# mdolab/adflow

Measured on NVIDIA H100. Metric: Mcells/s RANS-SA residual, higher is better.
Workload: dtype f64

## Files before the change

adflow_b200/csrc/adflow_b200.cu:

```cuda
#include <cuda_runtime.h>
#include <math.h>
#include <stdarg.h>
#include <stdio.h>
#include <string.h>

#include <map>
#include <string>
#include <vector>
#include <algorithm>

#include "adfb_common.cuh"
#include "state_kernels.cuh"
#include "residual_kernels.cuh"
#include "smoother_kernels.cuh"
#include "mg_kernels.cuh"
#include "ank_kernels.cuh"
#include "krylov_kernels.cuh"
#include "halo_kernels.cuh"
#include "dadi_kernels.cuh"
#include "sa_kernels.cuh"

namespace {

struct Block {
// ... 920 lines not shown
    static int mode = -1;
    if (mode < 0) { const char* e = getenv("ADFB_L2_PERSIST"); mode = e ? atoi(e) : 0; }
    static const void* current = nullptr;
    Block* only = nullptr;
    int nAlive = 0;
    for (Block& b : g.blocks) if (b.alive) { only = &b; nAlive++; }
    const void* want = (mode && nAlive == 1) ? (const void*)only->dev.w : nullptr;
    if (want == current) return;
    current = want;
    cudaStreamAttrValue av;
    memset(&av, 0, sizeof av);
    if (want) {
        int dev = 0, maxWin = 0, l2 = 0;
        cudaGetDevice(&dev);
        cudaDeviceGetAttribute(&maxWin, cudaDevAttrMaxAccessPolicyWindowSize, dev);
        cudaDeviceGetAttribute(&l2, cudaDevAttrMaxPersistingL2CacheSize, dev);
        size_t bytes = only->slabBytes;
        if ((size_t)maxWin < bytes) bytes = (size_t)maxWin;
        cudaDeviceSetLimit(cudaLimitPersistingL2CacheSize, (size_t)l2 < bytes ? (size_t)l2 : bytes);
        av.accessPolicyWindow.base_ptr = (void*)want;
        av.accessPolicyWindow.num_bytes = bytes;
        av.accessPolicyWindow.hitRatio = ((size_t)l2 >= bytes) ? 1.0f : (float)l2 / (float)bytes;
        av.accessPolicyWindow.hitProp = cudaAccessPropertyPersisting;
        av.accessPolicyWindow.missProp = cudaAccessPropertyStreaming;
    } else {
        av.accessPolicyWindow.num_bytes = 0;
    }
    cudaStreamSetAttribute(g.stream, cudaStreamAttributeAccessPolicyWindow, &av);
    cudaGetLastError();
}

static int residual_body(int level, unsigned flags) {
    static int overlapOn = -1;
    if (overlapOn < 0) { const char* e = getenv("ADFB_OVERLAP_BC"); overlapOn = e ? atoi(e) : 0; }
    static cudaStream_t s2 = nullptr;
    static cudaEvent_t eFork = nullptr, eJoin = nullptr;
    const bool preamble = !(flags & ADFB_RES_SKIP_PREAMBLE);
    const bool overlap = overlapOn && preamble && !g_kt.on && !overset_present(level);
    if (overlap && !s2) {
        CK(cudaStreamCreateWithFlags(&s2, cudaStreamNonBlocking));
        CK(cudaEventCreateWithFlags(&eFork, cudaEventDisableTiming));
        CK(cudaEventCreateWithFlags(&eJoin, cudaEventDisableTiming));
    }
    if (preamble) {
        for (Block& b : g.blocks) {
            if (!b.alive || b.level != level) continue;
            if (!g.mffdFuse && launch_state_prep(b.d, b.dev, g.prm, false, (flags & ADFB_RES_FLOW) != 0, g.stream)) return fail("state prep launch failed");
        }
        if (overlap) {
            CK(cudaEventRecord(eFork, g.stream));
            CK(cudaStreamWaitEvent(s2, eFork, 0));
            for (Block& b : g.blocks) {
                if (!b.alive || b.level != level) continue;
                if (launch_residual_core(b.d, b.dev, g.prm, flags, 1.0, 0, 1, s2, 0, RC_PREP_OWNED | RC_SA_INNER))
                    return fail("residual kernel launch failed: %s", cudaGetErrorString(cudaGetLastError()));
            }
            CK(cudaEventRecord(eJoin, s2));
        }
        const int nwLoc = g.prm.equations == ADFB_RANS ? 6 : 5;
        const bool fr = flags & ADFB_RES_FLOW, tr = (flags & ADFB_RES_TURB) && nwLoc == 6;
        const int lStart = fr ? 1 : 6, lEnd = tr ? 6 : 5;
        const bool ov = overset_present(level);
        const bool split = halo_split_ok(level);
        if (split && halo_exchange_impl(level, lStart, lEnd, 1, 1, ov, 1)) return 1;
        for (Block& b : g.blocks) {
            if (!b.alive || b.level != level) continue;
            if (launch_bc_levels(b.d, b.dev, b.subfaces, 1, g.prm.equations == ADFB_RANS && (flags & ADFB_RES_TURB), 1, g.stream))
                return fail("BC launch failed");
        }
        if (halo_exchange_impl(level, lStart, lEnd, 1, 1, ov, split ? 2 : 0)) return 1;
        if (ov) {
            for (Block& b : g.blocks) {
                if (!b.alive || b.level != level) continue;
                if (launch_bc_levels(b.d, b.dev, b.subfaces, 1, g.prm.equations == ADFB_RANS && (flags & ADFB_RES_TURB), 1, g.stream))
                    return fail("BC launch failed");
            }
        }
        if (overlap) CK(cudaStreamWaitEvent(g.stream, eJoin, 0));
    }
    const int rest = overlap ? (RC_PREP_HALO | RC_SA_SHELL | RC_FLOW) : RC_ALL;
    long long cell0 = 0;
    for (Block& b : g.blocks) {
        if (!b.alive || b.level != level) continue;
        const MffdEpi mf = {g.mffdFuse ? g.dMffd : nullptr, cell0};
        if (launch_residual_core(b.d, b.dev, g.prm, flags, 1.0, 0, 1, g.stream, 0, rest, mf))
            return fail("residual kernel launch failed: %s", cudaGetErrorString(cudaGetLastError()));
        cell0 += (long long)b.d.nx * b.d.ny * b.d.nz;
    }
    CK(cudaGetLastError());
    return 0;
}

static int nk_buffers(long long need) {
    if (g.nkN >= (size_t)need) return 0;
    for (double** p : {&g.nkA, &g.nkU, &g.nkF0, &g.nkY}) { if (*p) cudaFree(*p); *p = nullptr; }
    g.nkN = 0;
    g.nkHaveBase = false; g.ankHaveBase = false; g.ankTurbHaveBase = false;
    for (double** p : {&g.nkA, &g.nkU, &g.nkF0, &g.nkY}) CK(cudaMalloc((void**)p, need * sizeof(double)));
    if (!g.dRed) { CK(cudaMalloc((void**)&g.dRed, (2 * 1024 + 2) * sizeof(double))); g.dRedN = 2 * 1024 + 2; }
    g.nkN = need;
    return 0;
}
static int nk_vec_kernel(const double* vec, const double* base, double* out, double h, int mode) {
    long long off = 0;
    for (Block& b : g.blocks) {
        if (!b.alive || b.level != 1) continue;
        const long long n = (long long)b.d.nx * b.d.ny * b.d.nz * b.nw;
        KT_BEGIN(K_MFFD, g.stream);
        k_nkvec<<<(unsigned)((n + 255) / 256), 256, 0, g.stream>>>(b.d, b.dev, b.nw, vec ? vec + off : nullptr, base ? base + off : nullptr,
                                                                   out ? out + off : nullptr, h, mode, 0LL, LLONG_MAX);
        KT_END(K_MFFD, g.stream);
        off += n;
    }
    CK(cudaGetLastError());
    return 0;
}
static int nk_sumsq(const double* v, long long n, double* out) {
    const int nPart = 512;
    KT_BEGIN(K_MFFD, g.stream);
    k_sumsq_partial<<<nPart, 256, 0, g.stream>>>(v, n, g.dRed);
    KT_END(K_MFFD, g.stream);
    KT_BEGIN(K_MFFD, g.stream);
    k_sum_final<<<1, 256, 0, g.stream>>>(g.dRed, nPart);
    KT_END(K_MFFD, g.stream);
    if (g.nranks > 1) {
        const int rc = g.nccl.AllReduce(g.dRed + nPart, g.dRed + nPart, 1, kNcclDouble, kNcclSum, g.comm, g.stream);
        if (rc != 0) return fail("ncclAllReduce: %s", g.nccl.GetErrorString(rc));
    }
    CK(cudaMemcpyAsync(g.hRed, g.dRed + nPart, sizeof(double), cudaMemcpyDeviceToHost, g.stream));
    CK(cudaStreamSynchronize(g.stream));
    *out = g.hRed[0];
    return 0;
}
// ... 40 lines not shown
                acc += wgt[q];
                int e = (int)(acc / tot * nChunks + 0.5);
                if (e <= cb[q]) e = cb[q] + 1;
                if (e > nChunks - (S - 1 - q)) e = nChunks - (S - 1 - q);
                cb[q + 1] = e;
            }
            cb[S] = nChunks;
        }
        auto ownedEnd = [&](int chunkEnd) { return std::min(chunkEnd * kc, d.nz); };
        for (int q = 0; q < S; q++) {
            const long long q0 = (long long)ownedEnd(cb[q]) * plane, q1 = (long long)ownedEnd(cb[q + 1]) * plane;
            CK(cudaMemcpyAsync(g.nkA + off + q0, wVec + off + q0, (size_t)(q1 - q0) * sizeof(double), cudaMemcpyHostToDevice, g_ffIn));
            CK(cudaEventRecord(g_ffEv[0][q], g_ffIn));
        }
        int cNext = 0;
        for (int q = 0; q < S; q++) {
            const bool first = q == 0, last = q == S - 1;
            const int o0 = ownedEnd(cb[q]), o1 = ownedEnd(cb[q + 1]);
            CK(cudaStreamWaitEvent(sF, g_ffEv[0][q], 0));
            {
                const long long q0 = (long long)o0 * plane, q1 = (long long)o1 * plane;
                KT_BEGIN(K_MFFD, sF);
                k_nkvec<<<(unsigned)((q1 - q0 + 255) / 256), 256, 0, sF>>>(d, b.dev, b.nw, g.nkA + off, nullptr, nullptr, 0.0, 0, q0, q1);
                KT_END(K_MFFD, sF);
                dim3 tb(32, 4, 2);
                dim3 gr((d.nx + 31) / 32, (d.ny + 3) / 4, (o1 - o0 + 1) / 2);
                KT_BEGIN(K_STATE, sF);
                launch_pdl(k_state_prep, gr, tb, sF, d, b.dev, 0, rans ? 6 : 5, 1, o0, 1 + o1);
                KT_END(K_STATE, sF);
            }
            const int pLo = first ? 0 : 2 + o0, pHi = last ? d.kb : 1 + o1;
            if (launch_bc_levels(d, b.dev, b.subfaces, 1, rans ? 1 : 0, 1, sF, first ? -(1 << 30) : pLo, last ? (1 << 30) : pHi,
                                 (first ? 1 : 0) | (last ? 2 : 0)))
                return fail("BC launch failed");
            {
                dim3 tb(32, 4, 2);
                dim3 gr((d.NI + 31) / 32, (d.NJ + 3) / 4, (pHi - pLo + 2) / 2);
                KT_BEGIN(K_PREP, sF);
                launch_pdl(k_prep, gr, tb, sF, d, b.dev, 1, 1, 0, pLo, pHi);
                KT_END(K_PREP, sF);
            }
            int cEnd = cNext;
            while (cEnd < nChunks && (last || 2 + ownedEnd(cEnd + 1) - 1 + 2 <= pHi)) cEnd++;
            if (cEnd > cNext) {
                if (twoStreams) {
                    CK(cudaEventRecord(g_ffEv[2][q], sF));
                    CK(cudaStreamWaitEvent(sB, g_ffEv[2][q], 0));
                }
                const int r0 = ownedEnd(cNext), r1 = ownedEnd(cEnd);
                if (rans) {
                    dim3 tr(32, 4, 1);
                    dim3 gr((d.nx + 31) / 32, (d.ny + 3) / 4, r1 - r0);
                    KT_BEGIN(K_SA, sB);
                    k_sa<<<gr, tr, 0, sB>>>(d, b.dev, 0, MffdEpi{nullptr, 0}, r0, 1 + r1);
                    KT_END(K_SA, sB);
                }
                KT_BEGIN(K_RESID, sB);
                const int rc = launch_flowres_tile(d, b.dev, g.prm, (int)((b.dev.p - b.dev.w) / d.N), 1.0, 1, true, 0, sB, MffdEpi{nullptr, 0}, kc,
                                                   cNext, cEnd - cNext);
                KT_END(K_RESID, sB);
                if (rc) return fail("tile kernel launch failed inside the form-function pipeline");
                const long long q0 = (long long)r0 * plane, q1 = (long long)r1 * plane;
                KT_BEGIN(K_MFFD, sB);
                k_nkvec<<<(unsigned)((q1 - q0 + 255) / 256), 256, 0, sB>>>(d, b.dev, b.nw, nullptr, nullptr, g.nkY + off, 1.0, 2, q0, q1);
                KT_END(K_MFFD, sB);
                CK(cudaEventRecord(g_ffEv[1][q], sB));
                CK(cudaStreamWaitEvent(g_ffOut, g_ffEv[1][q], 0));
                CK(cudaMemcpyAsync(rVec + off + q0, g.nkY + off + q0, (size_t)(q1 - q0) * sizeof(double), cudaMemcpyDeviceToHost, g_ffOut));
                cNext = cEnd;
            }
        }
        off += (long long)d.nz * plane;
    }
    CK(cudaEventRecord(g_ffEv[3][1], g_ffIn));
    CK(cudaStreamWaitEvent(sF, g_ffEv[3][1], 0));
    CK(cudaEventRecord(g_ffEv[3][2], g_ffOut));
    CK(cudaStreamWaitEvent(sF, g_ffEv[3][2], 0));
    if (twoStreams) {
        CK(cudaEventRecord(g_ffEv[3][3], sB));
        CK(cudaStreamWaitEvent(sF, g_ffEv[3][3], 0));
    }
    CK(cudaGetLastError());
    return 0;
}
static int form_function_pipelined(const double* wVec, double* rVec, long long need) {
    (void)need;
    const int wantSlabs = form_function_pipe_slabs();
    if (wantSlabs < 2 || g.nranks > 1 || g_kt.on || g.mffdFuse) return -1;
    {
        auto busy = [](const std::map<int, Context::Pattern>& m) {
            auto it = m.find(1);
            return it != m.end() && it->second.set && (it->second.nSend || it->second.nRecv || it->second.nInt);
        };
        if (busy(g.pats) || busy(g.ovPats)) return -1;
    }
    if (!ff_pinned(wVec) || !ff_pinned(rVec)) return -1;
    for (Block& b : g.blocks) {
        if (!b.alive || b.level != 1) continue;
        if (!b.haveMetrics || b.nOrphans || !tile_kernel_applies(b.d, b.dev, g.prm) || b.d.nz < 16) return -1;
    }
    if (!g_ffIn) {
        CK(cudaStreamCreateWithFlags(&g_ffIn, cudaStreamNonBlocking));
        CK(cudaStreamCreateWithFlags(&g_ffOut, cudaStreamNonBlocking));
        CK(cudaStreamCreateWithFlags(&g_ffBack, cudaStreamNonBlocking));
        for (int a = 0; a < 4; a++) for (int q = 0; q < 34; q++) CK(cudaEventCreateWithFlags(&g_ffEv[a][q], cudaEventDisableTiming));
    }
    set_l2_window();
// ... 1101 lines not shown
```

adflow_b200/csrc/residual_kernels.cuh:

```cuda
#pragma once
#include "adfb_common.cuh"
#include <math.h>
#include <stdio.h>
#include <stdlib.h>
#include <string.h>
#include "fused_kernels.cuh"
#include "geom_cell.cuh"

#ifndef FACES_TPB
#define FACES_TPB 128
#endif
#ifndef FACES_MINB
#define FACES_MINB 4
#endif
#ifndef FACES_MINB_SPLIT
#define FACES_MINB_SPLIT 6
#endif
#ifndef SA_TPB
#define SA_TPB 128
#endif
#ifndef SA_MINB
#define SA_MINB 6
#endif
#ifndef NODAL_TPB
#define NODAL_TPB 256
#endif
#ifndef NODAL_MINB
#define NODAL_MINB 1
#endif
static inline dim3 tune_block(const char* env, dim3 dflt) {
    const char* e = getenv(env);
    if (!e) return dflt;
    int x = 0, y = 0, z = 0;
    if (sscanf(e, "%d,%d,%d", &x, &y, &z) == 3 && x > 0 && y > 0 && z > 0) return dim3(x, y, z);
    return dflt;
}

#define IRHO 0
#define IVX 1
#define IVY 2
#define IVZ 3
#define IRHOE 4
#define ITU1 5

namespace {

__global__ void __launch_bounds__(256) k_geom(Dims d, BlockDev b) {
    geom_cell(d, b, blockIdx.x * blockDim.x + threadIdx.x, blockIdx.y * blockDim.y + threadIdx.y, blockIdx.z * blockDim.z + threadIdx.z);
}

__global__ void __launch_bounds__(256) k_prep(Dims d, BlockDev b, int updateDt, int doRad, int part, int kOff, int kTop) {
    ADFB_PDL_SYNC();
    const int i = blockIdx.x * blockDim.x + threadIdx.x;
    const int j = blockIdx.y * blockDim.y + threadIdx.y;
    const int k = blockIdx.z * blockDim.z + threadIdx.z + kOff;
    if (i > d.ib || j > d.jb || k > d.kb || k > kTop) return;
    if (part) {
        const bool inner = i >= 3 && i < d.il && j >= 3 && j < d.jl && k >= 3 && k < d.kl;
        if (inner != (part == 1)) return;
    }
    const int N = (int)d.N, sJ = (int)d.sJ, sK = (int)d.sK;
    const int c = i + sJ * j + sK * k;
    const double gam = c_prm.gammaInf;
    const double rho = b.w[c], p = b.p[c];
    if (c_prm.spaceDiscr == ADFB_DISS_SCALAR) b.ss[c] = (c_prm.equations == ADFB_EULER) ? p : p * exp(-gam * log(rho));
    if (i < 1 || i > d.ie || j < 1 || j > d.je || k < 1 || k > d.ke) return;
    const bool viscous = c_prm.equations != ADFB_EULER;
    if (viscous) b.aa[c] = gam * p / rho;
    if (!doRad) return;

    const double clim2 = c_fheat[8];
    const double adis = c_prm.adis, asf = c_prm.acousticScaleFactor;
    const double ux = b.w[N + c], uy = b.w[2 * N + c], uz = b.w[3 * N + c];
    double cc2 = gam * p / rho;
    cc2 = dmax_(cc2, clim2);
    const double* ss = b.ssum;
    const double sxi = ss[c], syi = ss[N + c], szi = ss[2 * N + c];
    const double sxj = ss[3 * N + c], syj = ss[4 * N + c], szj = ss[5 * N + c];
    const double sxk = ss[6 * N + c], syk = ss[7 * N + c], szk = ss[8 * N + c];
    const double s2i = sxi * sxi + syi * syi + szi * szi;
    const double s2j = sxj * sxj + syj * syj + szj * szj;
    const double s2k = sxk * sxk + syk * syk + szk * szk;
    double ri = 0.5 * (fabs(ux * sxi + uy * syi + uz * szi) + asf * sqrt(cc2 * s2i));
    double rj = 0.5 * (fabs(ux * sxj + uy * syj + uz * szj) + asf * sqrt(cc2 * s2j));
    double rk = 0.5 * (fabs(ux * sxk + uy * syk + uz * szk) + asf * sqrt(cc2 * s2k));
    double dt = ri + rj + rk;
    if (b.coarse) {
        b.radI[c] = ri; b.radJ[c] = rj; b.radK[c] = rk;
    } else {
    ri = dmax_(ri, 1.e-25); rj = dmax_(rj, 1.e-25); rk = dmax_(rk, 1.e-25);
    const double li = log(ri), lj = log(rj), lk = log(rk);
    const double rij = exp(adis * (li - lj)), rjk = exp(adis * (lj - lk)), rik = rij * rjk;
    b.radI[c] = ri * (1.0 + 1.0 / rij + 1.0 / rik);
    b.radJ[c] = rj * (1.0 + 1.0 / rjk + rij);
    b.radK[c] = rk * (1.0 + rik + rjk);
    }

    if (!updateDt) return;
    if (i < 2 || i > d.il || j < 2 || j > d.jl || k < 2 || k > d.kl) return;
    if (viscous) {
        double rmu = b.rlv[c];
        rmu = rmu + b.rev[c];
        rmu = 0.5 * rmu / (rho * b.vol[c]);
        dt = dt + rmu * s2i;
        dt = dt + rmu * s2j;
        dt = dt + rmu * s2k;
    }
    const double plim = 0.001 * c_prm.pInfCorr;
    const double* pp = b.p;
    const double dpi = fabs(pp[c + 1] - 2.0 * p + pp[c - 1]) / (pp[c + 1] + 2.0 * p + pp[c - 1] + plim);
    const double dpj = fabs(pp[c + sJ] - 2.0 * p + pp[c - sJ]) / (pp[c + sJ] + 2.0 * p + pp[c - sJ] + plim);
    const double dpk = fabs(pp[c + sK] - 2.0 * p + pp[c - sK]) / (pp[c + sK] + 2.0 * p + pp[c - sK] + plim);
    const double rfl = 1.0 / (1.0 + 2.0 * (dpi + dpj + dpk));
    b.dtl[c] = rfl / dt;
}

__global__ void k_param_consts(double* out) {
    out[0] = ff_sslim_eval(c_prm);
    const double gam = c_prm.gammaInf;
    const double r0 = 1.0 / c_prm.wInf[0];
    out[1] = pow(c_prm.wInf[0], gam) / c_prm.pInfCorr;
    out[2] = sqrt(gam * c_prm.pInfCorr * r0);
}

template <bool GAOS>
__global__ void __launch_bounds__(NODAL_TPB, NODAL_MINB) k_nodal(Dims d, BlockDev b, int doGrad, int dissApprox) {
    ADFB_PDL_SYNC();
    const int i = blockIdx.x * blockDim.x + threadIdx.x + 1;
    const int j = blockIdx.y * blockDim.y + threadIdx.y + 1;
    const int k = blockIdx.z * blockDim.z + threadIdx.z + 1;
    if (i > d.ie || j > d.je || k > d.ke) return;
    const int N = (int)d.N, sJ = (int)d.sJ, sK = (int)d.sK;
    const int c = i + sJ * j + sK * k;
    if (c_prm.spaceDiscr == ADFB_DISS_SCALAR) {
        const double sslim = c_fheat[2];
        const double* ss = dissApprox ? b.shock : b.ss;
        const double s0 = ss[c];
        b.dss[c] = fabs((ss[c + 1] - 2.0 * s0 + ss[c - 1]) / (ss[c + 1] + 2.0 * s0 + ss[c - 1] + sslim));
        b.dss[N + c] = fabs((ss[c + sJ] - 2.0 * s0 + ss[c - sJ]) / (ss[c + sJ] + 2.0 * s0 + ss[c - sJ] + sslim));
        b.dss[2 * N + c] = fabs((ss[c + sK] - 2.0 * s0 + ss[c - sK]) / (ss[c + sK] + 2.0 * s0 + ss[c - sK] + sslim));
    } else if (c_prm.spaceDiscr == ADFB_DISS_MATRIX) {
        const double plim = 0.001 * c_prm.pInfCorr;
        const double* p = dissApprox ? b.shock : b.p;
        const double p0 = p[c];
        const int sdv[3] = {1, sJ, sK};
#pragma unroll
        for (int m = 0; m < 3; m++) {
            const double pp = p[c + sdv[m]], pm = p[c - sdv[m]];
            b.dss[m * N + c] = fabs((pp - 2.0 * p0 + pm) / (0.5 * (pp + 2.0 * p0 + pm) + 0.5 * (fabs(pp - p0) + fabs(p0 - pm)) + plim));
        }
    }
    if (!doGrad || i > d.il || j > d.jl || k > d.kl) return;
    double q[8][4];
#pragma unroll
    for (int m = 0; m < 8; m++) {
        const int cc = c + (m & 1) + ((m >> 1) & 1) * sJ + ((m >> 2) & 1) * sK;
        q[m][0] = b.w[N + cc]; q[m][1] = b.w[2 * N + cc]; q[m][2] = b.w[3 * N + cc]; q[m][3] = b.aa[cc];
    }
    double g[12];
#pragma unroll
    for (int m = 0; m < 12; m++) g[m] = 0.0;
    const int lo[3][4] = {{0, 2, 4, 6}, {0, 1, 4, 5}, {0, 1, 2, 3}};
    const int hi[3][4] = {{1, 3, 5, 7}, {2, 3, 6, 7}, {4, 5, 6, 7}};
    const int sd[3] = {1, sJ, sK};
#pragma unroll
    for (int dd = 2; dd >= 0; dd--) {
        const double* sv = b.sv + (3 * dd) * N;
// ... 339 lines not shown
}

template <bool VISCOUS, bool MERGED, int DISC, int APPROX, bool STOREWALL = false, int PART = 0, bool GAOS = false>
__global__ void __launch_bounds__(FACES_TPB, PART == 0 ? FACES_MINB : FACES_MINB_SPLIT) k_faces(Dims d, BlockDev b, double rFil, int doVisc, int doDiss) {
    ADFB_PDL_SYNC();
    const int i = blockIdx.x * blockDim.x + threadIdx.x + 1;
    const int j = blockIdx.y * blockDim.y + threadIdx.y + 1;
    const int k = blockIdx.z * blockDim.z + threadIdx.z + 1;
    if (i > d.il || j > d.jl || k > d.kl) return;
    const int N = (int)d.N, sJ = (int)d.sJ, sK = (int)d.sK;
    const int c = i + sJ * j + sK * k;
    const CellState m = load_cell(b, N, c);
    double fc[5], fd[5];
    double tq[9];
    double* const tqp = STOREWALL ? tq : nullptr;
    auto store_wall = [&](int dir, int side, long long pi) {
        double* dst = b.wallTau + ((long long)(dir * 2 + side) * 9) * b.wallP + pi;
#pragma unroll
        for (int l = 0; l < 9; l++) dst[l * b.wallP] = tq[l];
    };
    const bool oi = i >= 2, oj = j >= 2, ok = k >= 2;
    if (oj && ok) {
        face_flux<VISCOUS, DISC, APPROX, PART, GAOS>(b, N, c, 1, sJ, sK, 0, b.si, b.porI[c], b.radI, b.dss, m, rFil, doDiss, doVisc, fc, fd, tqp);
        if (STOREWALL && (i == 1 || i == d.il)) store_wall(0, i == 1 ? 0 : 1, j + (long long)d.NJ * k);
#pragma unroll
        for (int l = 0; l < 5; l++) {
            if (MERGED && PART == 2) b.flux[(15 + l) * N + c] = -fd[l];
            else if (MERGED) b.flux[l * N + c] = fc[l] - fd[l];
            else { b.flux[l * N + c] = fc[l]; b.flux[(5 + l) * N + c] = fd[l]; }
        }
    }
    if (oi && ok) {
        face_flux<VISCOUS, DISC, APPROX, PART, GAOS>(b, N, c, sJ, 1, sK, 1, b.sj, b.porJ[c], b.radJ, b.dss + N, m, rFil, doDiss, doVisc, fc, fd, tqp);
        if (STOREWALL && (j == 1 || j == d.jl)) store_wall(1, j == 1 ? 0 : 1, i + (long long)d.NI * k);
#pragma unroll
        for (int l = 0; l < 5; l++) {
            if (MERGED && PART == 2) b.flux[(20 + l) * N + c] = -fd[l];
            else if (MERGED) b.flux[(5 + l) * N + c] = fc[l] - fd[l];
            else { b.flux[(10 + l) * N + c] = fc[l]; b.flux[(15 + l) * N + c] = fd[l]; }
        }
    }
    if (oi && oj) {
        face_flux<VISCOUS, DISC, APPROX, PART, GAOS>(b, N, c, sK, 1, sJ, 2, b.sk, b.porK[c], b.radK, b.dss + 2 * N, m, rFil, doDiss, doVisc, fc, fd, tqp);
        if (STOREWALL && (k == 1 || k == d.kl)) store_wall(2, k == 1 ? 0 : 1, i + (long long)d.NI * j);
#pragma unroll
        for (int l = 0; l < 5; l++) {
            if (MERGED && PART == 2) b.flux[(25 + l) * N + c] = -fd[l];
            else if (MERGED) b.flux[(10 + l) * N + c] = fc[l] - fd[l];
            else { b.flux[(20 + l) * N + c] = fc[l]; b.flux[(25 + l) * N + c] = fd[l]; }
        }
    }
}

__device__ __forceinline__ double sa_adv_dir(const BlockDev& b, int N, int c, int sd, const double* __restrict__ ssum,
                                             double voli2, double ux, double uy, double uz) {
    const double* nt = b.w + ITU1 * N;
    const double xa = ssum[c] * voli2, ya = ssum[N + c] * voli2, za = ssum[2 * N + c] * voli2;
    const double uu = xa * ux + ya * uy + za * uz;
    double dwtx;
    if (uu > 0.0) {
        if (c_prm.secondOrdTurb) {
            const double dwtm1 = nt[c - sd] - nt[c - 2 * sd];
            const double dwt = nt[c] - nt[c - sd];
            const double dwtp1 = nt[c + sd] - nt[c];
            dwtx = dwt;
            if (dwt * dwtp1 > 0.0) dwtx = dwtx + 0.5 * ((fabs(dwt) < fabs(dwtp1)) ? dwt : dwtp1);
            if (dwt * dwtm1 > 0.0) dwtx = dwtx - 0.5 * ((fabs(dwt) < fabs(dwtm1)) ? dwt : dwtm1);
        } else {
            dwtx = nt[c] - nt[c - sd];
        }
    } else {
        if (c_prm.secondOrdTurb) {
            const double dwtm1 = nt[c] - nt[c - sd];
            const double dwt = nt[c + sd] - nt[c];
            const double dwtp1 = nt[c + 2 * sd] - nt[c + sd];
            dwtx = dwt;
            if (dwt * dwtp1 > 0.0) dwtx = dwtx - 0.5 * ((fabs(dwt) < fabs(dwtp1)) ? dwt : dwtp1);
            if (dwt * dwtm1 > 0.0) dwtx = dwtx + 0.5 * ((fabs(dwt) < fabs(dwtm1)) ? dwt : dwtm1);
        } else {
            dwtx = nt[c + sd] - nt[c];
        }
    }
    return uu * dwtx;
}

__device__ __forceinline__ double sa_visc_dir(const BlockDev& b, int N, int c, int sd, const double* __restrict__ s,
                                              const double* __restrict__ ssum, double nu, double acc) {
    const double* w = b.w;
    const double* vol = b.vol;
    const int cm = c - sd, cp = c + sd;
    const double cb3Inv = c_fheat[3] , cb2 = c_prm.rsaCb2;
    const double vc = vol[c];
    const double voli = 1.0 / vc;
    const double volmi = 2.0 / (vc + vol[cm]);
    const double volpi = 2.0 / (vc + vol[cp]);
    const double xm = s[cm] * volmi, ym = s[N + cm] * volmi, zm = s[2 * N + cm] * volmi;
    const double xp = s[c] * volpi, yp = s[N + c] * volpi, zp = s[2 * N + c] * volpi;
    const double xa = 0.5 * ssum[c] * voli, ya = 0.5 * ssum[N + c] * voli, za = 0.5 * ssum[2 * N + c] * voli;
    const double ttm = xm * xa + ym * ya + zm * za;
    const double ttp = xp * xa + yp * ya + zp * za;
    const double nt0 = w[ITU1 * N + c], ntm = w[ITU1 * N + cm], ntp = w[ITU1 * N + cp];
    const double cnud = -cb2 * nt0 * cb3Inv;
    const double cam = ttm * cnud, cap = ttp * cnud;
    const double nutm = 0.5 * (ntm + nt0), nutp = 0.5 * (ntp + nt0);
    const double num = 0.5 * (b.rlv[cm] / w[cm] + nu);
    const double nup = 0.5 * (b.rlv[cp] / w[cp] + nu);
    const double cdm = (num + (1.0 + cb2) * nutm) * ttm * cb3Inv;
    const double cdp = (nup + (1.0 + cb2) * nutp) * ttp * cb3Inv;
    const double c1m = dmax_(cdm + cam, 0.0), c1p = dmax_(cdp + cap, 0.0);
    const double c10 = c1m + c1p;
    return acc + c1m * ntm - c10 * nt0 + c1p * ntp;
}

__device__ __forceinline__ double sa_source(const BlockDev& b, int N, int sJ, int sK, int c, double nu) {
    const double* w = b.w;
    double gv[3][3];
#pragma unroll
    for (int v = 0; v < 3; v++) {
        const double* q = w + (IVX + v) * N;
        const double qip = q[c + 1], qim = q[c - 1], qjp = q[c + sJ], qjm = q[c - sJ], qkp = q[c + sK], qkm = q[c - sK];
#pragma unroll
        for (int m = 0; m < 3; m++) {
            const int o = m * N;
            gv[v][m] = qip * b.si[o + c] - qim * b.si[o + c - 1] + qjp * b.sj[o + c] - qjm * b.sj[o + c - sJ] +
                       qkp * b.sk[o + c] - qkm * b.sk[o + c - sK];
        }
    }
    const double fact = 0.25 / b.vol[c];
    const double sxx = 2.0 * fact * gv[0][0], syy = 2.0 * fact * gv[1][1], szz = 2.0 * fact * gv[2][2];
    const double sxy = fact * (gv[0][1] + gv[1][0]), sxz = fact * (gv[0][2] + gv[2][0]), syz = fact * (gv[1][2] + gv[2][1]);
    const double div2 = (2.0 * (1.0 / 3.0)) * ((sxx + syy + szz) * (sxx + syy + szz));
    const double strainMag2 = 2.0 * (sxy * sxy + sxz * sxz + syz * syz) + sxx * sxx + syy * syy + szz * szz;
    double sqrtProd;
    if (c_prm.turbProd == ADFB_PROD_STRAIN) {
        sqrtProd = sqrt(dmax_(2.0 * strainMag2 - div2, 1.e-25));
    } else {
        const double vortx = 2.0 * fact * (gv[2][1] - gv[1][2]);
        const double vorty = 2.0 * fact * (gv[0][2] - gv[2][0]);
        const double vortz = 2.0 * fact * (gv[1][0] - gv[0][1]);
        sqrtProd = sqrt(vortx * vortx + vorty * vorty + vortz * vortz);
    }
    const double cv13 = c_prm.rsaCv1 * c_prm.rsaCv1 * c_prm.rsaCv1;
    const double kar2Inv = c_fheat[4];
    const double cw3 = c_prm.rsaCw3;
    const double cw36 = (cw3 * cw3 * cw3) * (cw3 * cw3 * cw3);
    const double nt = w[ITU1 * N + c];
    const double dw_ = b.d2Wall[c];
    const double dist2Inv = 1.0 / (dw_ * dw_);
    const double chi = nt / nu, chi2 = chi * chi, chi3 = chi * chi2;
    const double fv1 = chi3 / (chi3 + cv13);
    const double fv2 = 1.0 - chi / (1.0 + chi * fv1);
    double ft2 = 0.0;
    if (c_prm.useft2SA) ft2 = c_prm.rsaCt3 * exp(-c_prm.rsaCt4 * chi2);
    double sst = sqrtProd + nt * fv2 * kar2Inv * dist2Inv;
    if (c_prm.useRotationSA) sst = sst + c_prm.rsaCrot * dmin_(0.0, sqrt(2.0 * strainMag2));
    sst = dmax_(sst, 1.e-10);
    double rr = nt * kar2Inv * dist2Inv / sst;
    rr = dmin_(rr, 10.0);
    const double rr2 = rr * rr, rr6 = rr2 * rr2 * rr2;
    const double gg = rr + c_prm.rsaCw2 * (rr6 - rr);
    const double gg2 = gg * gg, gg6 = gg2 * gg2 * gg2;
    const double termFw = pow((1.0 + cw36) / (gg6 + cw36), 1.0 / 6.0);
    const double fwSa = gg * termFw;
    const double term1 = c_prm.rsaCb1 * (1.0 - ft2) * sqrtProd * (c_prm.approxSA ? 0.0 : 1.0);
    const double term2 = dist2Inv * (kar2Inv * c_prm.rsaCb1 * ((1.0 - ft2) * fv2 + ft2) - c_prm.rsaCw1 * fwSa);
    return (term1 + term2 * nt) * nt;
}

__global__ void __launch_bounds__(SA_TPB, SA_MINB) k_sa(Dims d, BlockDev b, int part, MffdEpi mf, int kOff, int kTop) {
    const int i = blockIdx.x * blockDim.x + threadIdx.x + 2;
    const int j = blockIdx.y * blockDim.y + threadIdx.y + 2;
    const int k = blockIdx.z * blockDim.z + threadIdx.z + 2 + kOff;
    if (i > d.il || j > d.jl || k > d.kl || k > kTop) return;
    if (part) {
        const bool inner = i >= 4 && i <= d.il - 2 && j >= 4 && j <= d.jl - 2 && k >= 4 && k <= d.kl - 2;
        if (inner != (part == 1)) return;
    }
    const int N = (int)d.N, sJ = (int)d.sJ, sK = (int)d.sK;
    const int c = i + sJ * j + sK * k;
    const double rblank = dmax_((double)b.iblank[c], 0.0);
    const double nu = b.rlv[c] / b.w[c];
    double r = 0.0;
    r = r + sa_source(b, N, sJ, sK, c, nu);
    const double voli2 = 0.5 / b.vol[c];
    const double ux = b.w[N + c], uy = b.w[2 * N + c], uz = b.w[3 * N + c];
    r = r - sa_adv_dir(b, N, c, sK, b.ssum + 6 * N, voli2, ux, uy, uz);
    r = r - sa_adv_dir(b, N, c, sJ, b.ssum + 3 * N, voli2, ux, uy, uz);
    r = r - sa_adv_dir(b, N, c, 1, b.ssum, voli2, ux, uy, uz);
    r = sa_visc_dir(b, N, c, sK, b.sk, b.ssum + 6 * N, nu, r);
    r = sa_visc_dir(b, N, c, sJ, b.sj, b.ssum + 3 * N, nu, r);
    r = sa_visc_dir(b, N, c, 1, b.si, b.ssum, nu, r);
    const double dwv = -b.volRef[c] * r * rblank;
    b.dw[ITU1 * N + c] = dwv;
    if (mf.rec) mffd_epilogue(mf, d, i, j, k, ITU1, dwv, b.volRef[c], c_prm.turbResScale);
}

template <bool MERGED>
__global__ void __launch_bounds__(256) k_div(Dims d, BlockDev b, double rFil, int persistFw, int initWr) {
    ADFB_PDL_SYNC();
    const int i = blockIdx.x * blockDim.x + threadIdx.x + 2;
    const int j = blockIdx.y * blockDim.y + threadIdx.y + 2;
    const int k = blockIdx.z * blockDim.z + threadIdx.z + 2;
    if (i > d.il || j > d.jl || k > d.kl) return;
    const int N = (int)d.N, sJ = (int)d.sJ, sK = (int)d.sK;
    const int c = i + sJ * j + sK * k;
    const double rblank = dmax_((double)b.iblank[c], 0.0);
    const double* F = b.flux;
    if (MERGED) {
        const bool split = initWr == 2;
#pragma unroll
        for (int l = 0; l < 5; l++) {
            double a = 0.0;
            if (split) {
                a -= F[l * N + c - 1] + F[(15 + l) * N + c - 1];
                a += F[l * N + c] + F[(15 + l) * N + c];
                a -= F[(5 + l) * N + c - sJ] + F[(20 + l) * N + c - sJ];
                a += F[(5 + l) * N + c] + F[(20 + l) * N + c];
                a -= F[(10 + l) * N + c - sK] + F[(25 + l) * N + c - sK];
                a += F[(10 + l) * N + c] + F[(25 + l) * N + c];
            } else {
            a -= F[l * N + c - 1];
            a += F[l * N + c];
            a -= F[(5 + l) * N + c - sJ];
            a += F[(5 + l) * N + c];
            a -= F[(10 + l) * N + c - sK];
            a += F[(10 + l) * N + c];
            }
            b.dw[l * N + c] = a * rblank;
        }
    } else {
        const double sfil = 1.0 - rFil;
#pragma unroll
        for (int l = 0; l < 5; l++) {
            double a = initWr ? b.wr[l * N + c] : 0.0;
            a -= F[l * N + c - 1];
            a += F[l * N + c];
            a -= F[(10 + l) * N + c - sJ];
            a += F[(10 + l) * N + c];
            a -= F[(20 + l) * N + c - sK];
            a += F[(20 + l) * N + c];
            double fw = persistFw ? sfil * b.fw[l * N + c] : 0.0;
            fw += F[(5 + l) * N + c - 1];
            fw -= F[(5 + l) * N + c];
            fw += F[(15 + l) * N + c - sJ];
            fw -= F[(15 + l) * N + c];
            fw += F[(25 + l) * N + c - sK];
            fw -= F[(25 + l) * N + c];
            if (persistFw) b.fw[l * N + c] = fw;
            b.dw[l * N + c] = (a + fw) * rblank;
        }
    }
}

}

static int launch_geom(const Dims& d, const BlockDev& b, cudaStream_t stream) {
    dim3 tb(32, 4, 2);
    dim3 g((d.NI + tb.x - 1) / tb.x, (d.NJ + tb.y - 1) / tb.y, (d.NK + tb.z - 1) / tb.z);
    KT_BEGIN(K_METRICS, stream);
    k_geom<<<g, tb, 0, stream>>>(d, b);
    KT_END(K_METRICS, stream);
    return (int)cudaGetLastError();
}

static bool grad_aos() {
    static int v = -1;
    if (v < 0) { const char* e = getenv("ADFB_GRAD_AOS"); v = e ? atoi(e) : 0; }
    return v != 0;
}
static bool split_faces() {
    static int v = -1;
    if (v < 0) { const char* e = getenv("ADFB_SPLIT_FACES"); v = e ? atoi(e) : 0; }
    return v != 0;
}
static bool tile_kernel_applies(const Dims& d, const BlockDev& b, const AdfbParams& prm) {
    return fused_mode() > 0 && !b.coarse && prm.spaceDiscr == ADFB_DISS_SCALAR && !split_faces();
}
enum { RC_PREP_OWNED = 1, RC_PREP_HALO = 2, RC_SA_INNER = 4, RC_SA_SHELL = 8, RC_FLOW = 16, RC_ALL = 31 };
static int launch_residual_core(const Dims& d, const BlockDev& b, const AdfbParams& prm, unsigned flags, double rFil,
                                int persistFw, int doRad, cudaStream_t stream, int initWr = 0, int parts = RC_ALL,
                                MffdEpi mf = MffdEpi{nullptr, 0}) {
    const int flowRes = (flags & ADFB_RES_FLOW) != 0;
    const int turbRes = ((flags & ADFB_RES_TURB) != 0) && prm.equations == ADFB_RANS;
    const int updateDt = 1;
    const bool viscous = prm.equations != ADFB_EULER;
    const int doDiss = fabs(rFil) >= 1.e-10;
    const int doVisc = viscous && doDiss;
    const int dissApprox = (flags & ADFB_RES_DISS_APPROX) ? 1 : 0, viscApprox = (viscous && (flags & ADFB_RES_VISC_APPROX)) ? 1 : 0;
    if ((dissApprox || viscApprox) && persistFw) return 1;
    const bool gradAos = grad_aos() && flowRes && doVisc && !persistFw && !dissApprox && !viscApprox && !b.coarse && !split_faces() &&
                         !((flags & ADFB_RES_STORE_WALL) != 0) && prm.spaceDiscr == ADFB_DISS_SCALAR;
    dim3 tb(32, 4, 2);
    static cudaStream_t s_side = nullptr;
    static cudaEvent_t s_fork = nullptr, s_join = nullptr;
    static int s_conc = -1;
    if (s_conc < 0) {
        const char* e = getenv("ADFB_SA_CONCURRENT");
        s_conc = e ? atoi(e) : 1;
    }
    const int saPart = ((parts & RC_SA_INNER) && (parts & RC_SA_SHELL)) ? 0 : (parts & RC_SA_INNER) ? 1 : 2;
    const bool fork = turbRes && flowRes && s_conc && !g_kt.on && (parts & RC_FLOW);
    if (turbRes && (parts & (RC_SA_INNER | RC_SA_SHELL))) {
        dim3 tr = tune_block("ADFB_SA_BLOCK", dim3(32, 4, 1));
        dim3 g((d.nx + tr.x - 1) / tr.x, (d.ny + tr.y - 1) / tr.y, (d.nz + tr.z - 1) / tr.z);
        if (fork) {
            if (!s_side) {
                int prLo = 0, prHi = 0;
                cudaDeviceGetStreamPriorityRange(&prLo, &prHi);
                if (cudaStreamCreateWithPriority(&s_side, cudaStreamNonBlocking, prLo) != cudaSuccess) return 1;
                if (cudaEventCreateWithFlags(&s_fork, cudaEventDisableTiming) != cudaSuccess) return 1;
                if (cudaEventCreateWithFlags(&s_join, cudaEventDisableTiming) != cudaSuccess) return 1;
            }
            cudaStreamCopyAttributes(s_side, stream);
            cudaEventRecord(s_fork, stream);
            cudaStreamWaitEvent(s_side, s_fork, 0);
            k_sa<<<g, tr, 0, s_side>>>(d, b, saPart, mf, 0, INT_MAX);
            g_kt.launches++; g_kt.count[K_SA]++;
            cudaEventRecord(s_join, s_side);
        } else {
            KT_BEGIN(K_SA, stream);
            k_sa<<<g, tr, 0, stream>>>(d, b, saPart, mf, 0, INT_MAX);
            KT_END(K_SA, stream);
        }
    }
    if ((doRad || (flowRes && doDiss)) && (parts & (RC_PREP_OWNED | RC_PREP_HALO))) {
        const int prepPart = ((parts & RC_PREP_OWNED) && (parts & RC_PREP_HALO)) ? 0 : (parts & RC_PREP_OWNED) ? 1 : 2;
        dim3 g((d.NI + tb.x - 1) / tb.x, (d.NJ + tb.y - 1) / tb.y, (d.NK + tb.z - 1) / tb.z);
        KT_BEGIN(K_PREP, stream);
        launch_pdl(k_prep, g, tb, stream, d, b, updateDt, doRad, prepPart, 0, INT_MAX);
        KT_END(K_PREP, stream);
    }
    if (!(parts & RC_FLOW)) return (int)cudaGetLastError();
    bool fusedDone = false;
    static int fusedSmoother = -1;
    if (fusedSmoother < 0) { const char* e = getenv("ADFB_FUSED_SMOOTHER"); fusedSmoother = e ? atoi(e) : 0; }
    if (flowRes && fused_mode() > 0 && (!persistFw || fusedSmoother == 1 || (fusedSmoother == 2 && doDiss)) && !b.coarse && prm.spaceDiscr == ADFB_DISS_SCALAR && !dissApprox && !viscApprox && !initWr &&
        !(flags & ADFB_RES_STORE_WALL) && !split_faces()) {
        KT_BEGIN(K_RESID, stream);
        const int rc = launch_flowres_tile(d, b, prm, (int)((b.p - b.w) / d.N), rFil, doDiss, !persistFw, persistFw, stream, mf);
        KT_END(K_RESID, stream);
        if (rc > 0) return 1;
        fusedDone = rc == 0;
    }
    if (mf.rec && flowRes && !fusedDone) return 1;
    if (flowRes && doDiss && !fusedDone) {
        dim3 tn = tune_block("ADFB_NODAL_BLOCK", dim3(32, 4, 2));
        dim3 g((d.ie + tn.x - 1) / tn.x, (d.je + tn.y - 1) / tn.y, (d.ke + tn.z - 1) / tn.z);
        KT_BEGIN(K_NODAL, stream);
        if (gradAos) launch_pdl(k_nodal<true>, g, tn, stream, d, b, (int)(doVisc && !viscApprox), dissApprox);
        else launch_pdl(k_nodal<false>, g, tn, stream, d, b, (int)(doVisc && !viscApprox), dissApprox);
        KT_END(K_NODAL, stream);
    }
    if (flowRes && !fusedDone) {
        dim3 tr = tune_block("ADFB_FACES_BLOCK", dim3(32, 4, 1));
        dim3 g((d.il + tr.x - 1) / tr.x, (d.jl + tr.y - 1) / tr.y, (d.kl + tr.z - 1) / tr.z);
        const bool merged = !persistFw;
        KT_BEGIN(K_RESID, stream);
#define ADFB_LAUNCH_FACES(V, M, D, A) launch_pdl(k_faces<V, M, D, A>, g, tr, stream, d, b, rFil, doVisc, doDiss)
#define ADFB_FACES_DISC(V, M, A)                                           \
    do {                                                                   \
        if (prm.spaceDiscr == ADFB_DISS_SCALAR) ADFB_LAUNCH_FACES(V, M, ADFB_DISS_SCALAR, A); \
        else if (prm.spaceDiscr == ADFB_DISS_MATRIX) ADFB_LAUNCH_FACES(V, M, ADFB_DISS_MATRIX, A); \
        else ADFB_LAUNCH_FACES(V, M, ADFB_UPWIND, A);                       \
    } while (0)
        const int approx = dissApprox | (viscApprox << 1);
        int splitDone = 0;
        const bool storeWall = (flags & ADFB_RES_STORE_WALL) && viscous && doVisc && merged && approx == 0;
        if (b.coarse) {
            if (merged || approx) return 1;
            if (prm.spaceDiscrCoarse == ADFB_UPWIND) {
                if (viscous) launch_pdl(k_faces<true, false, ADFB_UPWIND, 1>, g, tr, stream, d, b, rFil, doVisc, doDiss);
                else launch_pdl(k_faces<false, false, ADFB_UPWIND, 1>, g, tr, stream, d, b, rFil, doVisc, doDiss);
            } else if (prm.spaceDiscrCoarse == ADFB_DISS_SCALAR) {
                if (viscous) launch_pdl(k_faces<true, false, ADFB_DISS_SCALAR, 4>, g, tr, stream, d, b, rFil, doVisc, doDiss);
                else launch_pdl(k_faces<false, false, ADFB_DISS_SCALAR, 4>, g, tr, stream, d, b, rFil, doVisc, doDiss);
            } else {
                if (viscous) launch_pdl(k_faces<true, false, ADFB_DISS_MATRIX, 4>, g, tr, stream, d, b, rFil, doVisc, doDiss);
                else launch_pdl(k_faces<false, false, ADFB_DISS_MATRIX, 4>, g, tr, stream, d, b, rFil, doVisc, doDiss);
            }
        } else if (storeWall) {
            if (prm.spaceDiscr == ADFB_DISS_SCALAR) launch_pdl(k_faces<true, true, ADFB_DISS_SCALAR, 0, true>, g, tr, stream, d, b, rFil, doVisc, doDiss);
            else if (prm.spaceDiscr == ADFB_DISS_MATRIX) launch_pdl(k_faces<true, true, ADFB_DISS_MATRIX, 0, true>, g, tr, stream, d, b, rFil, doVisc, doDiss);
            else launch_pdl(k_faces<true, true, ADFB_UPWIND, 0, true>, g, tr, stream, d, b, rFil, doVisc, doDiss);
        } else if (approx == 0 && viscous && merged && doVisc && split_faces()) {
            if (prm.spaceDiscr == ADFB_DISS_SCALAR) {
                launch_pdl(k_faces<true, true, ADFB_DISS_SCALAR, 0, false, 1>, g, tr, stream, d, b, rFil, doVisc, doDiss);
                launch_pdl(k_faces<true, true, ADFB_DISS_SCALAR, 0, false, 2>, g, tr, stream, d, b, rFil, doVisc, doDiss);
            } else if (prm.spaceDiscr == ADFB_DISS_MATRIX) {
                launch_pdl(k_faces<true, true, ADFB_DISS_MATRIX, 0, false, 1>, g, tr, stream, d, b, rFil, doVisc, doDiss);
                launch_pdl(k_faces<true, true, ADFB_DISS_MATRIX, 0, false, 2>, g, tr, stream, d, b, rFil, doVisc, doDiss);
            } else {
                launch_pdl(k_faces<true, true, ADFB_UPWIND, 0, false, 1>, g, tr, stream, d, b, rFil, doVisc, doDiss);
                launch_pdl(k_faces<true, true, ADFB_UPWIND, 0, false, 2>, g, tr, stream, d, b, rFil, doVisc, doDiss);
            }
            splitDone = 1;
        } else if (gradAos) {
            launch_pdl(k_faces<true, true, ADFB_DISS_SCALAR, 0, false, 0, true>, g, tr, stream, d, b, rFil, doVisc, doDiss);
        } else if (approx == 0) {
            if (viscous) { if (merged) ADFB_FACES_DISC(true, true, 0); else ADFB_FACES_DISC(true, false, 0); }
            else { if (merged) ADFB_FACES_DISC(false, true, 0); else ADFB_FACES_DISC(false, false, 0); }
        } else if (viscous) {
            if (approx == 1) ADFB_FACES_DISC(true, true, 1);
            else if (approx == 2) ADFB_FACES_DISC(true, true, 2);
            else ADFB_FACES_DISC(true, true, 3);
        } else {
            ADFB_FACES_DISC(false, true, 1);
        }
#undef ADFB_FACES_DISC
#undef ADFB_LAUNCH_FACES
        KT_END(K_RESID, stream);
        dim3 g2((d.nx + tb.x - 1) / tb.x, (d.ny + tb.y - 1) / tb.y, (d.nz + tb.z - 1) / tb.z);
        KT_BEGIN(K_DIV, stream);
        if (merged) launch_pdl(k_div<true>, g2, tb, stream, d, b, rFil, persistFw, splitDone ? 2 : 0);
        else launch_pdl(k_div<false>, g2, tb, stream, d, b, rFil, persistFw, initWr);
        KT_END(K_DIV, stream);
    }
    if (fork) cudaStreamWaitEvent(stream, s_join, 0);
    return (int)cudaGetLastError();
}
```

Measured before the change: 1393.

## Fuse SA turbulence residual with state prep kernel and drop side-stream fork

```diff
diff --git a/adflow_b200/csrc/adflow_b200.cu b/adflow_b200/csrc/adflow_b200.cu
--- a/adflow_b200/csrc/adflow_b200.cu
+++ b/adflow_b200/csrc/adflow_b200.cu
@@ -996,7 +996,7 @@
             CK(cudaStreamWaitEvent(s2, eFork, 0));
             for (Block& b : g.blocks) {
                 if (!b.alive || b.level != level) continue;
-                if (launch_residual_core(b.d, b.dev, g.prm, flags, 1.0, 0, 1, s2, 0, RC_PREP_OWNED | RC_SA_INNER))
+                if (launch_residual_core(b.d, b.dev, g.prm, flags, 1.0, 0, 1, s2, 0, RC_INNER))
                     return fail("residual kernel launch failed: %s", cudaGetErrorString(cudaGetLastError()));
             }
             CK(cudaEventRecord(eJoin, s2));
@@ -1022,7 +1022,7 @@
         }
         if (overlap) CK(cudaStreamWaitEvent(g.stream, eJoin, 0));
     }
-    const int rest = overlap ? (RC_PREP_HALO | RC_SA_SHELL | RC_FLOW) : RC_ALL;
+    const int rest = overlap ? (RC_SHELL | RC_FLOW) : RC_ALL;
     long long cell0 = 0;
     for (Block& b : g.blocks) {
         if (!b.alive || b.level != level) continue;
@@ -1169,7 +1169,7 @@
                     dim3 tr(32, 4, 1);
                     dim3 gr((d.nx + 31) / 32, (d.ny + 3) / 4, r1 - r0);
                     KT_BEGIN(K_SA, sB);
-                    k_sa<<<gr, tr, 0, sB>>>(d, b.dev, 0, MffdEpi{nullptr, 0}, r0, 1 + r1);
+                    k_sa<<<gr, tr, 0, sB>>>(d, b.dev, 0, 1, 1, 0, MffdEpi{nullptr, 0}, r0, 1 + r1);
                     KT_END(K_SA, sB);
                 }
                 KT_BEGIN(K_RESID, sB);
diff --git a/adflow_b200/csrc/residual_kernels.cuh b/adflow_b200/csrc/residual_kernels.cuh
--- a/adflow_b200/csrc/residual_kernels.cuh
+++ b/adflow_b200/csrc/residual_kernels.cuh
@@ -20,7 +20,7 @@
 #define SA_TPB 128
 #endif
 #ifndef SA_MINB
-#define SA_MINB 6
+#define SA_MINB 5
 #endif
 #ifndef NODAL_TPB
 #define NODAL_TPB 256
@@ -49,20 +49,13 @@
     geom_cell(d, b, blockIdx.x * blockDim.x + threadIdx.x, blockIdx.y * blockDim.y + threadIdx.y, blockIdx.z * blockDim.z + threadIdx.z);
 }
 
-__global__ void __launch_bounds__(256) k_prep(Dims d, BlockDev b, int updateDt, int doRad, int part, int kOff, int kTop) {
-    ADFB_PDL_SYNC();
-    const int i = blockIdx.x * blockDim.x + threadIdx.x;
-    const int j = blockIdx.y * blockDim.y + threadIdx.y;
-    const int k = blockIdx.z * blockDim.z + threadIdx.z + kOff;
-    if (i > d.ib || j > d.jb || k > d.kb || k > kTop) return;
-    if (part) {
-        const bool inner = i >= 3 && i < d.il && j >= 3 && j < d.jl && k >= 3 && k < d.kl;
-        if (inner != (part == 1)) return;
-    }
+struct CellOps { double r, u, v, w, rlv, vol, s[9]; };
+
+__device__ __forceinline__ void prep_cell(const Dims& d, const BlockDev& b, int i, int j, int k, int c, int updateDt, int doRad,
+                                          const CellOps* o) {
     const int N = (int)d.N, sJ = (int)d.sJ, sK = (int)d.sK;
-    const int c = i + sJ * j + sK * k;
     const double gam = c_prm.gammaInf;
-    const double rho = b.w[c], p = b.p[c];
+    const double rho = o ? o->r : b.w[c], p = b.p[c];
     if (c_prm.spaceDiscr == ADFB_DISS_SCALAR) b.ss[c] = (c_prm.equations == ADFB_EULER) ? p : p * exp(-gam * log(rho));
     if (i < 1 || i > d.ie || j < 1 || j > d.je || k < 1 || k > d.ke) return;
     const bool viscous = c_prm.equations != ADFB_EULER;
@@ -71,13 +64,15 @@
 
     const double clim2 = c_fheat[8];
     const double adis = c_prm.adis, asf = c_prm.acousticScaleFactor;
-    const double ux = b.w[N + c], uy = b.w[2 * N + c], uz = b.w[3 * N + c];
+    const double ux = o ? o->u : b.w[N + c], uy = o ? o->v : b.w[2 * N + c], uz = o ? o->w : b.w[3 * N + c];
     double cc2 = gam * p / rho;
     cc2 = dmax_(cc2, clim2);
-    const double* ss = b.ssum;
-    const double sxi = ss[c], syi = ss[N + c], szi = ss[2 * N + c];
-    const double sxj = ss[3 * N + c], syj = ss[4 * N + c], szj = ss[5 * N + c];
-    const double sxk = ss[6 * N + c], syk = ss[7 * N + c], szk = ss[8 * N + c];
+    double s[9];
+#pragma unroll
+    for (int m = 0; m < 9; m++) s[m] = o ? o->s[m] : b.ssum[m * N + c];
+    const double sxi = s[0], syi = s[1], szi = s[2];
+    const double sxj = s[3], syj = s[4], szj = s[5];
+    const double sxk = s[6], syk = s[7], szk = s[8];
     const double s2i = sxi * sxi + syi * syi + szi * szi;
     const double s2j = sxj * sxj + syj * syj + szj * szj;
     const double s2k = sxk * sxk + syk * syk + szk * szk;
@@ -99,9 +94,9 @@
     if (!updateDt) return;
     if (i < 2 || i > d.il || j < 2 || j > d.jl || k < 2 || k > d.kl) return;
     if (viscous) {
-        double rmu = b.rlv[c];
+        double rmu = o ? o->rlv : b.rlv[c];
         rmu = rmu + b.rev[c];
-        rmu = 0.5 * rmu / (rho * b.vol[c]);
+        rmu = 0.5 * rmu / (rho * (o ? o->vol : b.vol[c]));
         dt = dt + rmu * s2i;
         dt = dt + rmu * s2j;
         dt = dt + rmu * s2k;
@@ -113,6 +108,20 @@
     const double dpk = fabs(pp[c + sK] - 2.0 * p + pp[c - sK]) / (pp[c + sK] + 2.0 * p + pp[c - sK] + plim);
     const double rfl = 1.0 / (1.0 + 2.0 * (dpi + dpj + dpk));
     b.dtl[c] = rfl / dt;
+}
+
+__device__ __forceinline__ bool prep_inner(const Dims& d, int i, int j, int k) {
+    return i >= 3 && i < d.il && j >= 3 && j < d.jl && k >= 3 && k < d.kl;
+}
+
+__global__ void __launch_bounds__(256) k_prep(Dims d, BlockDev b, int updateDt, int doRad, int part, int kOff, int kTop) {
+    ADFB_PDL_SYNC();
+    const int i = blockIdx.x * blockDim.x + threadIdx.x;
+    const int j = blockIdx.y * blockDim.y + threadIdx.y;
+    const int k = blockIdx.z * blockDim.z + threadIdx.z + kOff;
+    if (i > d.ib || j > d.jb || k > d.kb || k > kTop) return;
+    if (part && prep_inner(d, i, j, k) != (part == 1)) return;
+    prep_cell(d, b, i, j, k, i + (int)d.sJ * j + (int)d.sK * k, updateDt, doRad, nullptr);
 }
 
 __global__ void k_param_consts(double* out) {
@@ -558,10 +567,10 @@
     }
 }
 
-__device__ __forceinline__ double sa_adv_dir(const BlockDev& b, int N, int c, int sd, const double* __restrict__ ssum,
+__device__ __forceinline__ double sa_adv_dir(const BlockDev& b, int N, int c, int sd, const double* ssum,
                                              double voli2, double ux, double uy, double uz) {
     const double* nt = b.w + ITU1 * N;
-    const double xa = ssum[c] * voli2, ya = ssum[N + c] * voli2, za = ssum[2 * N + c] * voli2;
+    const double xa = ssum[0] * voli2, ya = ssum[1] * voli2, za = ssum[2] * voli2;
     const double uu = xa * ux + ya * uy + za * uz;
     double dwtx;
     if (uu > 0.0) {
@@ -591,18 +600,17 @@
 }
 
 __device__ __forceinline__ double sa_visc_dir(const BlockDev& b, int N, int c, int sd, const double* __restrict__ s,
-                                              const double* __restrict__ ssum, double nu, double acc) {
+                                              const double* ssum, double vc, double nu, double acc) {
     const double* w = b.w;
     const double* vol = b.vol;
     const int cm = c - sd, cp = c + sd;
     const double cb3Inv = c_fheat[3] , cb2 = c_prm.rsaCb2;
-    const double vc = vol[c];
     const double voli = 1.0 / vc;
     const double volmi = 2.0 / (vc + vol[cm]);
     const double volpi = 2.0 / (vc + vol[cp]);
     const double xm = s[cm] * volmi, ym = s[N + cm] * volmi, zm = s[2 * N + cm] * volmi;
     const double xp = s[c] * volpi, yp = s[N + c] * volpi, zp = s[2 * N + c] * volpi;
-    const double xa = 0.5 * ssum[c] * voli, ya = 0.5 * ssum[N + c] * voli, za = 0.5 * ssum[2 * N + c] * voli;
+    const double xa = 0.5 * ssum[0] * voli, ya = 0.5 * ssum[1] * voli, za = 0.5 * ssum[2] * voli;
     const double ttm = xm * xa + ym * ya + zm * za;
     const double ttp = xp * xa + yp * ya + zp * za;
     const double nt0 = w[ITU1 * N + c], ntm = w[ITU1 * N + cm], ntp = w[ITU1 * N + cp];
@@ -618,7 +626,7 @@
     return acc + c1m * ntm - c10 * nt0 + c1p * ntp;
 }
 
-__device__ __forceinline__ double sa_source(const BlockDev& b, int N, int sJ, int sK, int c, double nu) {
+__device__ __forceinline__ double sa_source(const BlockDev& b, int N, int sJ, int sK, int c, double nu, double vol) {
     const double* w = b.w;
     double gv[3][3];
 #pragma unroll
@@ -632,7 +640,7 @@
                        qkp * b.sk[o + c] - qkm * b.sk[o + c - sK];
         }
     }
-    const double fact = 0.25 / b.vol[c];
+    const double fact = 0.25 / vol;
     const double sxx = 2.0 * fact * gv[0][0], syy = 2.0 * fact * gv[1][1], szz = 2.0 * fact * gv[2][2];
     const double sxy = fact * (gv[0][1] + gv[1][0]), sxz = fact * (gv[0][2] + gv[2][0]), syz = fact * (gv[1][2] + gv[2][1]);
     const double div2 = (2.0 * (1.0 / 3.0)) * ((sxx + syy + szz) * (sxx + syy + szz));
@@ -673,32 +681,54 @@
     return (term1 + term2 * nt) * nt;
 }
 
-__global__ void __launch_bounds__(SA_TPB, SA_MINB) k_sa(Dims d, BlockDev b, int part, MffdEpi mf, int kOff, int kTop) {
-    const int i = blockIdx.x * blockDim.x + threadIdx.x + 2;
-    const int j = blockIdx.y * blockDim.y + threadIdx.y + 2;
-    const int k = blockIdx.z * blockDim.z + threadIdx.z + 2 + kOff;
-    if (i > d.il || j > d.jl || k > d.kl || k > kTop) return;
-    if (part) {
-        const bool inner = i >= 4 && i <= d.il - 2 && j >= 4 && j <= d.jl - 2 && k >= 4 && k <= d.kl - 2;
-        if (inner != (part == 1)) return;
-    }
+__device__ __forceinline__ void sa_row(const Dims& d, const BlockDev& b, int i, int j, int k, int c, const MffdEpi& mf,
+                                       CellOps& o) {
     const int N = (int)d.N, sJ = (int)d.sJ, sK = (int)d.sK;
-    const int c = i + sJ * j + sK * k;
     const double rblank = dmax_((double)b.iblank[c], 0.0);
-    const double nu = b.rlv[c] / b.w[c];
+    o.r = b.w[c]; o.rlv = b.rlv[c]; o.vol = b.vol[c];
+    const double nu = o.rlv / o.r;
     double r = 0.0;
-    r = r + sa_source(b, N, sJ, sK, c, nu);
-    const double voli2 = 0.5 / b.vol[c];
-    const double ux = b.w[N + c], uy = b.w[2 * N + c], uz = b.w[3 * N + c];
-    r = r - sa_adv_dir(b, N, c, sK, b.ssum + 6 * N, voli2, ux, uy, uz);
-    r = r - sa_adv_dir(b, N, c, sJ, b.ssum + 3 * N, voli2, ux, uy, uz);
-    r = r - sa_adv_dir(b, N, c, 1, b.ssum, voli2, ux, uy, uz);
-    r = sa_visc_dir(b, N, c, sK, b.sk, b.ssum + 6 * N, nu, r);
-    r = sa_visc_dir(b, N, c, sJ, b.sj, b.ssum + 3 * N, nu, r);
-    r = sa_visc_dir(b, N, c, 1, b.si, b.ssum, nu, r);
+    r = r + sa_source(b, N, sJ, sK, c, nu, o.vol);
+    const double voli2 = 0.5 / o.vol;
+    o.u = b.w[N + c]; o.v = b.w[2 * N + c]; o.w = b.w[3 * N + c];
+    auto ssum = [&](int dir) {
+        for (int m = 3 * dir; m < 3 * dir + 3; m++) o.s[m] = b.ssum[m * N + c];
+        return o.s + 3 * dir;
+    };
+    r = r - sa_adv_dir(b, N, c, sK, ssum(2), voli2, o.u, o.v, o.w);
+    r = r - sa_adv_dir(b, N, c, sJ, ssum(1), voli2, o.u, o.v, o.w);
+    r = r - sa_adv_dir(b, N, c, 1, ssum(0), voli2, o.u, o.v, o.w);
+    r = sa_visc_dir(b, N, c, sK, b.sk, o.s + 6, o.vol, nu, r);
+    r = sa_visc_dir(b, N, c, sJ, b.sj, o.s + 3, o.vol, nu, r);
+    r = sa_visc_dir(b, N, c, 1, b.si, o.s, o.vol, nu, r);
     const double dwv = -b.volRef[c] * r * rblank;
     b.dw[ITU1 * N + c] = dwv;
     if (mf.rec) mffd_epilogue(mf, d, i, j, k, ITU1, dwv, b.volRef[c], c_prm.turbResScale);
+}
+
+__device__ __forceinline__ bool sa_inner(const Dims& d, int i, int j, int k) {
+    return i >= 4 && i <= d.il - 2 && j >= 4 && j <= d.jl - 2 && k >= 4 && k <= d.kl - 2;
+}
+
+__global__ void __launch_bounds__(SA_TPB, SA_MINB) k_sa(Dims d, BlockDev b, int withPrep, int updateDt, int doRad, int part,
+                                                        MffdEpi mf, int kOff, int kTop) {
+    ADFB_PDL_SYNC();
+    const int o0 = withPrep ? 0 : 2;
+    const int i = (int)(blockIdx.x * blockDim.x + threadIdx.x) + 2 - (withPrep ? (int)blockDim.x : 0);
+    const int j = blockIdx.y * blockDim.y + threadIdx.y + o0;
+    const int k = blockIdx.z * blockDim.z + threadIdx.z + o0 + kOff;
+    if (i < 0 || i > d.ib || j > d.jb || k > d.kb || k > kTop) return;
+    const bool owned = i >= 2 && i <= d.il && j >= 2 && j <= d.jl && k >= 2 && k <= d.kl;
+    const bool prep = withPrep && (!part || prep_inner(d, i, j, k) == (part == 1));
+    const bool sa = owned && (!part || sa_inner(d, i, j, k) == (part == 1));
+    const int c = i + (int)d.sJ * j + (int)d.sK * k;
+    CellOps o;
+    if (sa) {
+        sa_row(d, b, i, j, k, c, mf, o);
+        if (prep) prep_cell(d, b, i, j, k, c, updateDt, doRad, &o);
+    } else if (prep) {
+        prep_cell(d, b, i, j, k, c, updateDt, doRad, nullptr);
+    }
 }
 
 template <bool MERGED>
@@ -782,7 +812,7 @@
 static bool tile_kernel_applies(const Dims& d, const BlockDev& b, const AdfbParams& prm) {
     return fused_mode() > 0 && !b.coarse && prm.spaceDiscr == ADFB_DISS_SCALAR && !split_faces();
 }
-enum { RC_PREP_OWNED = 1, RC_PREP_HALO = 2, RC_SA_INNER = 4, RC_SA_SHELL = 8, RC_FLOW = 16, RC_ALL = 31 };
+enum { RC_INNER = 1, RC_SHELL = 2, RC_FLOW = 4, RC_ALL = 7 };
 static int launch_residual_core(const Dims& d, const BlockDev& b, const AdfbParams& prm, unsigned flags, double rFil,
                                 int persistFw, int doRad, cudaStream_t stream, int initWr = 0, int parts = RC_ALL,
                                 MffdEpi mf = MffdEpi{nullptr, 0}) {
@@ -797,43 +827,17 @@
     const bool gradAos = grad_aos() && flowRes && doVisc && !persistFw && !dissApprox && !viscApprox && !b.coarse && !split_faces() &&
                          !((flags & ADFB_RES_STORE_WALL) != 0) && prm.spaceDiscr == ADFB_DISS_SCALAR;
     dim3 tb(32, 4, 2);
-    static cudaStream_t s_side = nullptr;
-    static cudaEvent_t s_fork = nullptr, s_join = nullptr;
-    static int s_conc = -1;
-    if (s_conc < 0) {
-        const char* e = getenv("ADFB_SA_CONCURRENT");
-        s_conc = e ? atoi(e) : 1;
-    }
-    const int saPart = ((parts & RC_SA_INNER) && (parts & RC_SA_SHELL)) ? 0 : (parts & RC_SA_INNER) ? 1 : 2;
-    const bool fork = turbRes && flowRes && s_conc && !g_kt.on && (parts & RC_FLOW);
-    if (turbRes && (parts & (RC_SA_INNER | RC_SA_SHELL))) {
-        dim3 tr = tune_block("ADFB_SA_BLOCK", dim3(32, 4, 1));
-        dim3 g((d.nx + tr.x - 1) / tr.x, (d.ny + tr.y - 1) / tr.y, (d.nz + tr.z - 1) / tr.z);
-        if (fork) {
-            if (!s_side) {
-                int prLo = 0, prHi = 0;
-                cudaDeviceGetStreamPriorityRange(&prLo, &prHi);
-                if (cudaStreamCreateWithPriority(&s_side, cudaStreamNonBlocking, prLo) != cudaSuccess) return 1;
-                if (cudaEventCreateWithFlags(&s_fork, cudaEventDisableTiming) != cudaSuccess) return 1;
-                if (cudaEventCreateWithFlags(&s_join, cudaEventDisableTiming) != cudaSuccess) return 1;
-            }
-            cudaStreamCopyAttributes(s_side, stream);
-            cudaEventRecord(s_fork, stream);
-            cudaStreamWaitEvent(s_side, s_fork, 0);
-            k_sa<<<g, tr, 0, s_side>>>(d, b, saPart, mf, 0, INT_MAX);
-            g_kt.launches++; g_kt.count[K_SA]++;
-            cudaEventRecord(s_join, s_side);
+    if ((doRad || (flowRes && doDiss) || turbRes) && (parts & (RC_INNER | RC_SHELL))) {
+        const int part = ((parts & RC_INNER) && (parts & RC_SHELL)) ? 0 : (parts & RC_INNER) ? 1 : 2;
+        KT_BEGIN(K_PREP, stream);
+        if (turbRes) {
+            const dim3 tr(32, SA_TPB / 32, 1);
+            const dim3 g(1 + (d.ib + tr.x - 2) / tr.x, (d.NJ + tr.y - 1) / tr.y, d.NK);
+            launch_pdl(k_sa, g, tr, stream, d, b, 1, updateDt, doRad, part, mf, 0, INT_MAX);
         } else {
-            KT_BEGIN(K_SA, stream);
-            k_sa<<<g, tr, 0, stream>>>(d, b, saPart, mf, 0, INT_MAX);
-            KT_END(K_SA, stream);
-        }
-    }
-    if ((doRad || (flowRes && doDiss)) && (parts & (RC_PREP_OWNED | RC_PREP_HALO))) {
-        const int prepPart = ((parts & RC_PREP_OWNED) && (parts & RC_PREP_HALO)) ? 0 : (parts & RC_PREP_OWNED) ? 1 : 2;
-        dim3 g((d.NI + tb.x - 1) / tb.x, (d.NJ + tb.y - 1) / tb.y, (d.NK + tb.z - 1) / tb.z);
-        KT_BEGIN(K_PREP, stream);
-        launch_pdl(k_prep, g, tb, stream, d, b, updateDt, doRad, prepPart, 0, INT_MAX);
+            const dim3 g((d.NI + tb.x - 1) / tb.x, (d.NJ + tb.y - 1) / tb.y, (d.NK + tb.z - 1) / tb.z);
+            launch_pdl(k_prep, g, tb, stream, d, b, updateDt, doRad, part, 0, INT_MAX);
+        }
         KT_END(K_PREP, stream);
     }
     if (!(parts & RC_FLOW)) return (int)cudaGetLastError();
@@ -921,6 +925,5 @@
         else launch_pdl(k_div<false>, g2, tb, stream, d, b, rFil, persistFw, initWr);
         KT_END(K_DIV, stream);
     }
-    if (fork) cudaStreamWaitEvent(stream, s_join, 0);
     return (int)cudaGetLastError();
 }
```

Measured after the change: 1411, median of 6. 1.01x the previous value.
